# LDeakin/VkVolume

Hardware: AMD Instinct MI355X
Metric: Mray/s (higher is better)
Workload: dtype f32

## Files before the change

### vkvolume_amd/csrc/capi.hip

```cpp
#include <cmath>
#include <cstdarg>
#include <cstdio>
#include <cstdlib>
#include <cstring>
#include <dlfcn.h>
#include <mutex>
#include <new>

#include <algorithm>
#include <exception>
#include <string>
#include <vector>

#include "../host/load_volume.h"
#include "../host/vkv_math.hpp"
#include "vkv_device.hpp"
#include "../../include/vkvolume_amd_debug.h"

namespace vkv
{
int launch_gradient_map(vkv_ctx *, const uint8_t *, uint8_t *, VkvExtent3D, const VkvTransferFunctionUniform *, hipStream_t);
int launch_occupancy_map(vkv_ctx *, const uint8_t *, const uint8_t *, const uint8_t *, const VkvTransferFunctionUniform *, VkvExtent3D, uint8_t *,
                         VkvExtent3D, hipStream_t, uint32_t *d_bits, bool bits_ready = false);
int launch_distance_map(vkv_ctx *, uint8_t *, uint8_t *, VkvExtent3D, hipStream_t);
int launch_distance_map_anisotropic(vkv_ctx *, uint8_t *const[8], uint8_t *, VkvExtent3D, hipStream_t);
int launch_synth_volume(vkv_ctx *, uint8_t *, VkvExtent3D, uint32_t, uint32_t, hipStream_t);
int launch_scatter_tiles_frames(vkv_ctx *, uint32_t, void *const *, const void *const *, const VkvTileRect *, const uint32_t *, uint32_t, uint32_t, uint32_t, uint32_t, uint32_t,
                                uint32_t, hipStream_t);
void screen_tile_rect(const VkvRayCastUniform *, const VkvRayGen *, uint32_t, uint32_t, uint32_t, uint32_t, uint32_t, VkvTileRect *);
int prepare_render(vkv_ctx *, const VkvRenderParams *, uint32_t, hipStream_t);
// ... 93 lines not shown
			{
				void *q = nullptr;
				if (hipMalloc(&q, kScratchBytes) == hipSuccess)
				{
					ctx->overflow_scratch.push_back(q);
					p = static_cast<uint8_t *>(q);
				}
			}
			if (p)
			{
				b = new (std::nothrow) vkv_ctx::ScratchBlock;
				if (b)
				{
					b->p = p;
					ctx->scratch_blocks.emplace_back(b);
				}
			}
			if (!b)
			{
				set_error(ctx, VKV_E_UNSUPPORTED, "no scratch block left for a new stream: the arena reserves %zu (call vkv_prepare_render for the stream at set-up "
				                                  "time, give finished streams back with vkv_release_stream, or raise VKV_ARENA_BYTES)", ctx->table_base / kScratchBytes);
				return StreamScratch{};
			}
			ctx->scratch.emplace(key, b);
		}
	}
	StreamScratch r;
	r.lock = std::unique_lock<std::mutex>(b->lock);
	r.p    = b->p;
	return r;
}

static bool table_upload(vkv_ctx *ctx, vkv_ctx::Table &t, hipStream_t s, bool setup)
{
	const size_t bytes = t.host.size() * sizeof(uint32_t);
	bool         from_arena = false;
	t.d                = static_cast<uint32_t *>(arena_take_table(ctx, bytes, setup, &from_arena));
	if (!t.d)
		return false;
	if (hipEventCreateWithFlags(&t.uploaded, hipEventDisableTiming) != hipSuccess)
		return false;
	const void *src = t.host.data();
	if (from_arena && ctx->table_mirror)
	{
// ... 23 lines not shown
{
	if (t.ready)
		return t.d;
	if (setup ? hipEventSynchronize(t.uploaded) == hipSuccess : hipEventQuery(t.uploaded) == hipSuccess)
	{
		t.ready = true;
		return t.d;
	}
	if ((s != t.upload_stream || s == hipStreamPerThread) && hipStreamWaitEvent(s, t.uploaded, 0) != hipSuccess)
		return nullptr;
	return t.d;
}

constexpr size_t kMaxCachedTables = 1024;

const uint32_t *packed_addr_lut(vkv_ctx *ctx, int W, int H, int D, uint32_t *lut_y, uint32_t *lut_z, uint32_t *words, hipStream_t stream, bool setup)
{
	std::lock_guard<std::mutex> lock(ctx->mutex);
	for (auto *t : ctx->addr_luts)
		if (t->W == W && t->H == H && t->D == D)
		{
			*lut_y = t->lut_y, *lut_z = t->lut_z, *words = t->words;
			return table_on_stream(t->table, stream, setup);
		}
	if (ctx->addr_luts.size() >= kMaxCachedTables)
		return nullptr;
	const PackedDims pd  = packed_dims(W, H, D);
	const uint32_t   nmx = (uint32_t) (W + 1) / 32 + 1, nmy = (uint32_t) (H + 1) / 32 + 1, nmz = (uint32_t) (D + 1) / 32 + 1;
	const uint32_t   ny = 96 + nmx, nz = (ny + nmy + 1) & ~1u, total = nz + 2 * nmz;
	auto *           e  = new (std::nothrow) vkv_ctx::AddrLut{W, H, D, ny, nz, total, {}};
	if (!e)
		return nullptr;
	std::vector<uint32_t> &h = e->table.host;
	h.assign(total, 0u);
	for (uint32_t j = 0; j < 32; ++j)
	{
		h[j]      = (((j >> 2) & 7u) << 8) + (j & 3u) * 2u;
		h[32 + j] = (((j >> 2) & 7u) << 11) + (j & 3u) * 10u;
		h[64 + j] = (((j >> 2) & 7u) << 14) + (j & 3u) * 50u;
	}
	for (uint32_t m = 0; m < nmx; ++m)
		h[96 + m] = m << 17;
	for (uint32_t m = 0; m < nmy; ++m)
		h[ny + m] = (m * (uint32_t) pd.mx) << 17;
	for (uint32_t m = 0; m < nmz; ++m)
	{
		const uint64_t z = ((uint64_t) m * (uint64_t) pd.my * (uint64_t) pd.mx) << 17;
		h[nz + 2 * m] = (uint32_t) z, h[nz + 2 * m + 1] = (uint32_t) (z >> 32);
	}
	if (!table_upload(ctx, e->table, stream, setup))
	{
		delete e;
		return nullptr;
	}
	ctx->addr_luts.push_back(e);
	*lut_y = ny, *lut_z = nz, *words = total;
	return e->table.d;
}

const uint32_t *tile_start_order(vkv_ctx *ctx, uint32_t img_w, uint32_t img_h, uint32_t tile_w, uint32_t tile_h, uint32_t first, uint32_t stride, uint32_t count,
                                 hipStream_t stream, bool setup)
{
	if (count < 2)
		return nullptr;
	const uint32_t tiles_x = (img_w + tile_w - 1) / tile_w, tiles_y = (img_h + tile_h - 1) / tile_h;
	std::lock_guard<std::mutex> lock(ctx->mutex);
	const float mix_heavy_f = ctx->tuning.tile_mix_heavy, mix_spread_f = ctx->tuning.tile_mix_spread;
	for (auto *t : ctx->tile_orders)
		if (t->tiles_x == tiles_x && t->tiles_y == tiles_y && t->tile_w == tile_w && t->tile_h == tile_h && t->img_w == img_w && t->img_h == img_h && t->first == first &&
		    t->stride == stride && t->count == count && t->mix_heavy == mix_heavy_f && t->mix_spread == mix_spread_f)
			return table_on_stream(t->table, stream, setup);
// ... 282 lines not shown
			ctx->table_mirror = static_cast<uint8_t *>(m);
		void *cp = nullptr, *cd = nullptr;
		if (hipHostMalloc(&cp, (size_t) kCaptureSlots * kCaptureSlotBytes, hipHostMallocDefault) == hipSuccess &&
		    hipMalloc(&cd, (size_t) kCaptureSlots * kCaptureSlotBytes) == hipSuccess)
		{
			ctx->capture_pool = static_cast<uint8_t *>(cp), ctx->capture_pool_device = static_cast<uint8_t *>(cd);
			for (uint32_t i = 0; i < kCaptureSlots; ++i)
			{
				vkv_ctx::CaptureSlot c;
				c.pinned = ctx->capture_pool + (size_t) i * kCaptureSlotBytes, c.device = ctx->capture_pool_device + (size_t) i * kCaptureSlotBytes, c.pooled = true;
				ctx->capture_slots.push_back(c);
			}
		}
		else if (cp)
			(void) hipHostFree(cp);
	}
	*out_ctx      = ctx;
	return VKV_OK;
}

void vkv_destroy(vkv_ctx *ctx)
{
	if (!ctx)
		return;
	{
		DeviceGuard guard(ctx->device);
		(void) hipDeviceSynchronize();
		drop_tables(ctx);
		for (auto *f : ctx->feedback)
		{
			(void) hipFree(f->d_cost);
			(void) hipFree(f->d_order);
					delete f;
		}
		for (void *p : ctx->overflow_scratch)
			(void) hipFree(p);
		drop_capture_blocks(ctx);
		if (ctx->capture_pool)
			(void) hipHostFree(ctx->capture_pool);
		if (ctx->capture_pool_device)
			(void) hipFree(ctx->capture_pool_device);
		if (ctx->table_mirror)
			(void) hipHostFree(ctx->table_mirror);
		(void) hipFree(ctx->arena);
	}
	delete ctx;
}

int vkv_get_tuning(const vkv_ctx *ctx, VkvTuning *out)
{
	if (!ctx || !out)
		return VKV_E_INVALID_ARGUMENT;
// ... 680 lines not shown
	if (!P->d_out_color && !P->d_out_rgba8 && !P->d_out_counts && !P->d_out_depth)
		return set_error(ctx, VKV_E_INVALID_ARGUMENT, "render: no output buffer");
	return VKV_OK;
}

static void build_alpha_lut(const VkvTransferFunctionUniform &tf, float *lut)
{
	const float sf_inv = 1.0f / tf.sampling_factor;
	for (int a = 0; a < 256; ++a)
	{
		const float v = tf.voxel_alpha_factor * (1.0f - std::pow(1.0f - (float) a / 255.0f, sf_inv));
		lut[a]        = std::min(std::max(v, 0.0f), 1.0f);
	}
}

int vkv_render(vkv_ctx *ctx, const VkvRenderParams *P, void *stream)
{
	if (!ctx)
		return VKV_E_INVALID_ARGUMENT;
	DeviceGuard guard(ctx->device);
	const int   rc = check_render_params(ctx, P);
	if (rc != VKV_OK)
		return rc;
	float lut[256];
	build_alpha_lut(P->transfer_function, lut);
	return launch_render(ctx, P, lut, (hipStream_t) stream);
}

int vkv_render_batch(vkv_ctx *ctx, const VkvRenderParams *P, uint32_t count, void *stream)
{
	if (!ctx)
		return VKV_E_INVALID_ARGUMENT;
	DeviceGuard guard(ctx->device);
	if (!P || count == 0 || count > VKV_MAX_BATCH)
		return set_error(ctx, VKV_E_INVALID_ARGUMENT, "render_batch: count must be 1 .. %d", VKV_MAX_BATCH);
	std::vector<float> luts((size_t) count * 256);
	for (uint32_t i = 0; i < count; ++i)
	{
		const int rc = check_render_params(ctx, &P[i]);
		if (rc != VKV_OK)
			return rc;
		const VkvRenderParams &a = P[i], &b = P[0];
		if (a.options.skipping_type != b.options.skipping_type || (a.options.early_ray_termination != 0) != (b.options.early_ray_termination != 0) ||
		    (a.transfer_function.use_gradient != 0) != (b.transfer_function.use_gradient != 0) ||
		    (a.use_precomputed_gradient != 0) != (b.use_precomputed_gradient != 0))
			return set_error(ctx, VKV_E_INVALID_ARGUMENT, "render_batch: frame %u needs a different kernel variant than frame 0", i);
		build_alpha_lut(a.transfer_function, luts.data() + (size_t) i * 256);
	}
	return launch_render_batch(ctx, P, count, luts.data(), (hipStream_t) stream);
}

static bool resolve_rect(const VkvTileRect *rect, uint32_t image_width, uint32_t image_height, uint32_t tile_width, uint32_t tile_height, VkvTileRect &out)
{
	const uint32_t tiles_x = (image_width + tile_width - 1) / tile_width, tiles_y = (image_height + tile_height - 1) / tile_height;
	if (!rect || rect->w == 0 || rect->h == 0)
	{
		out = VkvTileRect{0u, 0u, tiles_x, tiles_y};
		return true;
	}
	out = *rect;
	return (uint64_t) rect->x0 + rect->w <= tiles_x && (uint64_t) rect->y0 + rect->h <= tiles_y;
}
// ... 224 lines not shown
```

### vkvolume_amd/csrc/raymarch.hip

```cpp
#include <algorithm>
#include <cmath>
#include <cstdio>
#include <cstdlib>
#include <cstring>
#include <mutex>
#include <new>
#include <vector>

#include "raymarch_inst.hpp"

constexpr int kCostBins = 1024;

__device__ __forceinline__ void tile_order_from_cost(uint32_t *__restrict__ cost, uint32_t *__restrict__ order_out, uint32_t count)
{
	__shared__ uint32_t s_bin[kCostBins];
	constexpr int       kPerThread = 40;
	for (int b = threadIdx.x; b < kCostBins; b += blockDim.x)
		s_bin[b] = 0;
	__syncthreads();
	for (uint32_t base = 0; base < count; base += 256u * kPerThread)
	{
		uint32_t c[kPerThread];
#pragma unroll
		for (int j = 0; j < kPerThread; ++j)
// ... 83 lines not shown
	if (A.order_out)
		tile_order_from_cost(A.tile_cost, A.order_out, A.tile_count);
}

namespace vkv
{

LeanChoice choose_lean(const RayMarchArgs &a, const VkvTuning &T)
{
	const size_t lut_bytes = (size_t) a.lut_words * sizeof(uint32_t);
	if (!a.packed || !a.addr_lut || lut_bytes > kMaxLutBytes || !map_fits_u24((uint32_t) a.mw, (uint32_t) a.mh, (uint32_t) a.md))
		return {0, lean_lds_bytes(0, 0, a.W, a.H, a.D)};
	const bool        no_full  = T.address_tables < 2;
	const size_t      full_end = kFullLutWord * 4 + full_lut_bytes(a.W, a.H, a.D);
	const bool        fits_u32 = packed_bytes(packed_dims(a.W, a.H, a.D)) <= (1ull << 33);
	if (!no_full && fits_u32 && full_end <= (size_t) T.full_table_lds_limit)
		return {2, lean_lds_bytes(2, a.lut_words, a.W, a.H, a.D)};
	return {1, lean_lds_bytes(1, a.lut_words, a.W, a.H, a.D)};
}

static int launch_single(vkv_ctx *ctx, int skip, bool ert, int sched, const VkvTuning &T, int grad, RayMarchArgs &a, hipStream_t s)
{
	switch (skip)
	{
		case VKV_SKIP_NONE: return ert ? RayMarchLaunchers<VKV_SKIP_NONE, true>::single(ctx, sched, T, grad, a, s) : RayMarchLaunchers<VKV_SKIP_NONE, false>::single(ctx, sched, T, grad, a, s);
		case VKV_SKIP_BLOCK: return ert ? RayMarchLaunchers<VKV_SKIP_BLOCK, true>::single(ctx, sched, T, grad, a, s) : RayMarchLaunchers<VKV_SKIP_BLOCK, false>::single(ctx, sched, T, grad, a, s);
		case VKV_SKIP_DISTANCE: return ert ? RayMarchLaunchers<VKV_SKIP_DISTANCE, true>::single(ctx, sched, T, grad, a, s) : RayMarchLaunchers<VKV_SKIP_DISTANCE, false>::single(ctx, sched, T, grad, a, s);
		case VKV_SKIP_ANISOTROPIC_DISTANCE:
			return ert ? RayMarchLaunchers<VKV_SKIP_ANISOTROPIC_DISTANCE, true>::single(ctx, sched, T, grad, a, s) : RayMarchLaunchers<VKV_SKIP_ANISOTROPIC_DISTANCE, false>::single(ctx, sched, T, grad, a, s);
		default: return set_error(ctx, VKV_E_INVALID_ARGUMENT, "render: bad skipping_type %d", skip);
	}
// ... 218 lines not shown
	a.back        = (int) std::ceil(P->transfer_function.sampling_factor);
	a.clamp_always = T.clamp_always != 0 ? 1u : 0u;
	{
		double vx = 0.0, vy = 0.0;
		const double dim[3] = {(double) a.W, (double) a.H, (double) a.D};
		for (int k = 0; k < 3; ++k)
			vx += (double) a.ddx[k] * dim[k] * (double) a.ddx[k] * dim[k], vy += (double) a.ddy[k] * dim[k] * (double) a.ddy[k] * dim[k];
		const double r = (vx > 0.0 && vy > 0.0) ? std::sqrt(vx / vy) : 1.0;
		a.wave_pw_log2 = T.wave_shape == 4 ? 2u : (T.wave_shape == 8 ? 3u : (T.wave_shape == 16 ? 4u : (r >= 1.6 ? 2u : (r <= 1.0 / 1.6 ? 4u : 3u))));
	}
	{
		const float m[3] = {(float) a.mw, (float) a.mh, (float) a.md};
		for (int k = 0; k < 3; ++k)
			a.mapf[k] = m[k], a.mapb[k] = std::nextafterf(m[k], 0.0f);
	}
	a.addr_lut = nullptr, a.lut_y = a.lut_z = a.lut_words = 0;
	if (a.packed && T.address_tables != 0)
		a.addr_lut = packed_addr_lut(ctx, a.W, a.H, a.D, &a.lut_y, &a.lut_z, &a.lut_words, s, setup);
	screen_bound_of_box(a, T);
	a.tile_order = (T.tile_order_linear || !whole_schedule) ? nullptr
	                                                         : tile_start_order(ctx, a.img_w, a.img_h, a.tile_w, a.tile_h, a.tile_first, a.tile_stride, a.tile_count, s, setup);
	a.order_h = 0;
	if (!whole_schedule && !T.tile_order_linear && a.tile_first == 0 && a.tile_stride == 1 && (uint64_t) a.tile_count == (uint64_t) a.tiles_x * P->tiles.rect.h)
		a.order_h = P->tiles.rect.h;
	for (int i = 0; i < 256; ++i)
		a.alpha_lut[i] = alpha_lut[i];
	return VKV_OK;
}

static bool apply_feedback(vkv_ctx *ctx, RayMarchArgs &a, hipStream_t s)
{
	(void) s;
	const void *      target = a.out_rgba8 ? (const void *) a.out_rgba8 : (const void *) a.out_color;
// ... 96 lines not shown
			rc = fill_render_args(ctx, &P[i], lut, a, s, T, true, true);
		if (rc != VKV_OK)
			return rc;
		load_render_code(P[i].options.skipping_type, P[i].options.early_ray_termination != 0);
	}
	load_feedback_code();
	if (!stream_scratch(ctx, s, true).p)
		return VKV_E_UNSUPPORTED;
	return VKV_OK;
}

int launch_render_batch(vkv_ctx *ctx, const VkvRenderParams *P, uint32_t n, const float *alpha_luts, hipStream_t s)
{
	static_assert(kMaxBatch * sizeof(RayMarchArgs) <= kScratchBytes - kBatchArgsOffset, "batch argument blocks must fit the stream scratch");
	static_assert(kPullHeadsBytes + kMaxBatch * sizeof(RayMarchArgs) <= kCaptureSlotBytes, "a captured launch's upload must fit its pinned slot");
	const VkvTuning           T = tuning_of(ctx);
	std::vector<RayMarchArgs> host(n);
	for (uint32_t i = 0; i < n; ++i)
	{
		const int rc = fill_render_args(ctx, &P[i], alpha_luts + (size_t) i * 256, host[i], s, T, false, true);
		if (rc != VKV_OK)
			return rc;
		if (!host[i].packed)
			return set_error(ctx, VKV_E_INVALID_ARGUMENT, "render_batch: frame %u has no packed sampling image (d_packed_volume)", i);
		if (host[i].blocks_per_tile != host[0].blocks_per_tile)
			return set_error(ctx, VKV_E_INVALID_ARGUMENT, "render_batch: frame %u has a different tile size than frame 0", i);
		if (ctx->d_debug_orders && i < ctx->debug_order_frames && ctx->debug_order_count == host[i].tile_count)
			host[i].tile_order = ctx->d_debug_orders + (size_t) i * ctx->debug_order_count;
	}
	uint32_t max_tiles = 0, ref = 0;
	bool     same_count = true;
	for (uint32_t i = n; i-- > 0;)
	{
		max_tiles = std::max(max_tiles, host[i].nblocks ? host[i].tile_count : 0u);
		if (host[i].nblocks)
			ref = i;
	}
	if (max_tiles == 0)
		return VKV_OK;
	for (uint32_t i = 0; i < n; ++i)
		same_count = same_count && host[i].nblocks != 0 && host[i].tile_count == max_tiles;
	bool any_sort = false;
	for (uint32_t i = 0; i < n && P[0].options.early_ray_termination != 0; ++i)
		any_sort = apply_feedback(ctx, host[i], s) || any_sort;
	const StreamScratch scratch = stream_scratch(ctx, s);
	if (!scratch.p)
		return VKV_E_UNSUPPORTED;
	RayMarchArgs *   d_frames = reinterpret_cast<RayMarchArgs *>(scratch.p + kBatchArgsOffset);
	uint32_t *       d_heads  = reinterpret_cast<uint32_t *>(scratch.p + kBatchArgsOffset - kPullHeadsBytes);
	std::vector<uint8_t> upload(kPullHeadsBytes + n * sizeof(RayMarchArgs), 0);
	std::memcpy(upload.data() + kPullHeadsBytes, host.data(), n * sizeof(RayMarchArgs));
	const void *upload_src = upload.data();
	struct SlotGuard
	{
		vkv_ctx *ctx;
		size_t   index;
		bool     armed;
		~SlotGuard()
		{
			if (!armed)
				return;
			std::lock_guard<std::mutex> lock(ctx->mutex);
			if (index < ctx->capture_slots.size())
				ctx->capture_slots[index].in_use = false, ctx->capture_slots[index].owner = VkvStreamKey{};
		}
	} slot_guard{ctx, 0, false};
	{
		hipStreamCaptureStatus capture = hipStreamCaptureStatusNone;
		if (hipStreamIsCapturing(s, &capture) == hipSuccess && capture == hipStreamCaptureStatusActive)
		{
			std::lock_guard<std::mutex> lock(ctx->mutex);
			vkv_ctx::CaptureSlot *      slot = nullptr;
			for (auto &c : ctx->capture_slots)
				if (!c.in_use)
				{
					slot = &c;
					break;
				}
			if (!slot)
			{
				vkv_ctx::CaptureSlot c;
				void *               hp = nullptr, *dp = nullptr;
				hipStreamCaptureMode mode = hipStreamCaptureModeRelaxed;
				(void) hipThreadExchangeStreamCaptureMode(&mode);
				const hipError_t ea = hipHostMalloc(&hp, kCaptureSlotBytes, hipHostMallocDefault);
				const hipError_t eb = ea == hipSuccess ? hipMalloc(&dp, kCaptureSlotBytes) : ea;
				const bool failed = ea != hipSuccess || eb != hipSuccess || !hp || !dp;
				if (failed && hp)
					(void) hipHostFree(hp);
				(void) hipThreadExchangeStreamCaptureMode(&mode);
				if (failed)
					return set_error(ctx, VKV_E_UNSUPPORTED, "render_batch: no argument block for a captured launch: %s", hipGetErrorString(ea != hipSuccess ? ea : eb));
				c.pinned = static_cast<uint8_t *>(hp), c.device = static_cast<uint8_t *>(dp);
				ctx->capture_slots.push_back(c);
				slot = &ctx->capture_slots.back();
			}
			slot->in_use = true, slot->owner = stream_key(s);
			slot_guard.index = (size_t) (slot - ctx->capture_slots.data()), slot_guard.armed = true;
			std::memcpy(slot->pinned, upload.data(), upload.size());
			upload_src = slot->pinned;
			d_heads    = reinterpret_cast<uint32_t *>(slot->device);
			d_frames   = reinterpret_cast<RayMarchArgs *>(slot->device + kPullHeadsBytes);
		}
	}
	const hipError_t e = hipMemcpyAsync(d_heads, upload_src, upload.size(), hipMemcpyHostToDevice, s);
	if (e != hipSuccess)
		return set_error(ctx, (int) e, "render_batch: argument upload: %s", hipGetErrorString(e));
	const uint64_t grid = (uint64_t) ((max_tiles + 7u) / 8u) * 8u * host[0].blocks_per_tile * n;
	if (grid > 0x7fffffffull)
		return set_error(ctx, VKV_E_UNSUPPORTED, "render_batch: too many workgroups for one launch");
	const bool ert  = P[0].options.early_ray_termination != 0;
	const int  grad = !P[0].transfer_function.use_gradient ? 0 : (P[0].use_precomputed_gradient ? 1 : 2);
	const bool        sequential = T.batch_sequential != 0;
	const uint32_t    gpf        = sequential ? (uint32_t) (grid / n / 8) : 0u;
	LeanChoice        choice     = choose_lean(host[ref], T);
	bool              no_counts  = true;
	for (uint32_t i = 0; i < n; ++i)
		no_counts = no_counts && (host[i].nblocks == 0 || !wants_counts(host[i]));
	for (uint32_t i = 0; i < n; ++i)
	{
		if (i == ref || host[i].nblocks == 0)
			continue;
// ... 33 lines not shown
```

### vkvolume_amd/csrc/raymarch_core.hpp

```cpp
#pragma once

#include <type_traits>

#include "vkv_device.hpp"

using namespace vkv;

constexpr int kTraceWords = 10;
constexpr uint32_t kFillPerTile = 3;

struct RayMarchArgs
{
	float dir00[3], ddx[3], ddy[3];
	float cam[3];
	float plane_tex[4];
	float block_size[3];
	float model[16], view[16], proj[16];
	float view_proj_inv[16], model_inv[16];
	float sampling_factor, grad_modifier;
	int W, H, D, mw, mh, md;
	const uint8_t * vol, *grad, *tf;
	const uint8_t * packed;
	int             pmx, pmy;
	const uint32_t *tf_bits;
// ... 5 lines not shown
	const float *   in_depth;
	uint32_t        depth_attachment, blend;
	uint32_t        img_w, img_h, tile_w, tile_h, tiles_x, tile_first, tile_stride, tile_count, compact;
	uint32_t        org_x, org_y;
	uint32_t        fill_tiles, img_tiles_x, rect_tx0, rect_ty0, rect_th;
	uint32_t        fill_rgba8_rows;
	uint32_t        blocks_per_tile_x, blocks_per_tile, nblocks;
	int             test;
	unsigned long long *trace;
	int             back;
	uint32_t        clamp_always;
	float           mapf[3], mapb[3];
	uint32_t        wave_pw_log2;
	const uint32_t *addr_lut;
	uint32_t        lut_y, lut_z, lut_words;
	uint32_t        cull_x0, cull_x1, cull_y0, cull_y1;
	const uint32_t *tile_order;
	uint32_t        order_h;
	uint32_t *      queue_heads;
	uint32_t *      tile_cost;
	uint32_t *      order_out;
	float           alpha_lut[256];
};

struct Ray
{
	float          ex, ey, ez;
	float          sx, sy, sz;
	float          six, siy, siz;
	const uint8_t *dmap;
// ... 697 lines not shown
			float    unorm[256];
		} g;
		struct
		{
			float  ai[258], ag[258];
			float2 pair[256];
		} s;
	};
};

__device__ __forceinline__ bool tf_is_separable(const RayMarchArgs &A)
{
	return A.tf_bits != nullptr && (A.tf_bits[kTfFlagWord] & kTfFlagSeparable) != 0u;
}

__device__ __forceinline__ bool stage_tables_er(const RayMarchArgs &A, RmLds &L)
{
	const bool sep = tf_is_separable(A);
	for (int i = threadIdx.x; i < 256; i += blockDim.x)
	{
		const float a = A.alpha_lut[i];
		if (!sep)
			L.g.alpha[i] = a;
		if (sep)
		{
			L.s.ai[i]   = __uint_as_float(A.tf_bits[kTfAiWord + i]);
			L.s.ag[i]   = __uint_as_float(A.tf_bits[kTfAgWord + i]);
			if (i == 255)
				L.s.ai[256] = L.s.ai[255], L.s.ag[256] = L.s.ag[255];
			L.s.pair[i] = i == 0 ? make_float2(0.0f, 0.0f) : make_float2(a, unorm8(i) * a);
		}
		else
			L.g.unorm[i] = unorm8(i);
	}
	if (!sep && A.tf_bits)
		for (int i = threadIdx.x; i < 2048; i += blockDim.x)
			L.g.bits[i] = A.tf_bits[i];
	__syncthreads();
	return sep;
}
template <int W>
__device__ __forceinline__ bool block_pixel(const RayMarchArgs &A, uint32_t b, uint32_t rb, uint32_t &px, uint32_t &py, uint32_t &o)
{
	constexpr uint32_t G = 64 / W;
	uint32_t           bx, by;
	const uint32_t     wb = rb / G, g = rb % G;
	if (W == 1)
	{
		const uint32_t pwl = A.wave_pw_log2, pprl = 4u - pwl;
		bx = ((wb & ((1u << pprl) - 1u)) << pwl) + (g & ((1u << pwl) - 1u));
		by = ((wb >> pprl) << (6u - pwl)) + (g >> pwl);
	}
	else
// ... 163 lines not shown
}

constexpr uint32_t kFullLutWord  = 1028;
__host__ __device__ __forceinline__ bool map_fits_u24(uint32_t mw, uint32_t mh, uint32_t md) { return (uint64_t) mh * md < (1ull << 24) && mw < (1u << 24); }
constexpr size_t   kFullLdsLimit = 17920;

__host__ __device__ __forceinline__ size_t full_lut_bytes(int W, int H, int D) { return (size_t) (W + 2 + H + 2 + D + 2) * 4; }

__host__ __forceinline__ size_t lean_lds_bytes(int kind, uint32_t lut_words, int W, int H, int D)
{
	const size_t two_level = kLdsBase + sizeof(RmLds) + (size_t) lut_words * 4;
	if (kind == 0)
		return kLdsBase + sizeof(RmLds);
	if (kind == 1)
		return two_level;
	const size_t full_end = kLdsBase + (size_t) kFullLutWord * 4 + full_lut_bytes(W, H, D);
	return two_level > full_end ? two_level : full_end;
}

__device__ __forceinline__ uint32_t *full_lut_base(const RmLds &L) { return const_cast<uint32_t *>(reinterpret_cast<const uint32_t *>(&L)) + kFullLutWord; }

__device__ __forceinline__ void stage_full_lut(const RayMarchArgs &A, RmLds &L)
{
	static_assert(sizeof(((RmLds *) nullptr)->s) == kFullLutWord * 4, "full tables start behind the separable TF tables");
	const uint32_t  nx = (uint32_t) A.W + 2u, ny = (uint32_t) A.H + 2u, nz = (uint32_t) A.D + 2u;
	uint32_t *      fx = full_lut_base(L), *fy = fx + nx, *fz = fy + ny;
	const uint32_t *g  = A.addr_lut;
	for (uint32_t b = threadIdx.x; b < nx; b += blockDim.x)
		fx[b] = (g[b & 31u] + g[kLutXm + (b >> 5)]) >> 1;
	for (uint32_t b = threadIdx.x; b < ny; b += blockDim.x)
		fy[b] = (g[32u + (b & 31u)] + g[A.lut_y + (b >> 5)]) >> 1;
	for (uint32_t b = threadIdx.x; b < nz; b += blockDim.x)
		fz[b] = (uint32_t) ((((((uint64_t) g[A.lut_z + 2u * (b >> 5) + 1u]) << 32) | g[A.lut_z + 2u * (b >> 5)]) + g[64u + (b & 31u)]) >> 1);
}

struct FullLutConsts
{
	float          w, h, d, oy, oz;
	const uint8_t *base;
};

template <bool SCALAR = false>
__device__ __forceinline__ FullLutConsts full_lut_consts(const RayMarchArgs &A)
{
	FullLutConsts c;
	c.w = (float) A.W, c.h = (float) A.H, c.d = (float) A.D;
	c.base = A.packed;
	c.oy = (float) (4 * (A.W + 2) + 4);
// ... 482 lines not shown
	R.o = o;
	const unsigned long long t_start = A.trace ? __builtin_amdgcn_s_memrealtime() : 0ull;
	const unsigned long long c_start = A.trace ? __builtin_amdgcn_s_memtime() : 0ull;
	bool marched = false;
	if (inside)
	{
		if (px >= A.cull_x0 && px <= A.cull_x1 && py >= A.cull_y0 && py <= A.cull_y1)
			marched = ray_setup<SKIP>(A, px, py, R);
		else
			ray_clear(R);
	}
	uint32_t  iter  = 0;
	LeanStamp stamp = {};
	if (wg_any(marched))
	{
		if ((LF & kLeanLut) != 0 && PACKED && GRAD != 2)
		{
			if ((LF & kLeanFull) != 0 && tf_is_separable(A))
				stage_full_lut(A, L);
			else
				stage_addr_lut(A);
		}
		const bool sep = stage_tables_er(A, L);
		if (marched)
		{
			if (sep)
			{
				constexpr bool kSafe = (LF & kLeanSafe) != 0 && (LF & kLeanFull) != 0 && PACKED && GRAD != 2 && SKIP != VKV_SKIP_NONE && (LF & kLeanStamp) == 0;
				if constexpr (kSafe)
				{
					if (lean_free_wave(A, R))
						lean_march<SKIP, ERT, GRAD, PACKED, true, LF, true>(A, R, L, iter, stamp);
					else
						lean_march<SKIP, ERT, GRAD, PACKED, true, LF>(A, R, L, iter, stamp);
				}
				else
					lean_march<SKIP, ERT, GRAD, PACKED, true, LF>(A, R, L, iter, stamp);
			}
// ... 138 lines not shown
				rec[0] = t_start, rec[1] = t_end, rec[2] = it, rec[3] = ((unsigned long long) __builtin_amdgcn_s_getreg((3 << 11) | 20) << 32) | (rank * upt + w);
				rec[4] = t_setup, rec[5] = t_march;
				for (int x = 6; x < kTraceWords; ++x)
					rec[x] = 0;
			}
		}
	}
}

template <int SKIP, bool ERT, int GRAD, uint32_t LF>
__global__ void __launch_bounds__(256) __attribute__((amdgpu_waves_per_eu(8, 8))) k_raymarch_lean_pull(const RayMarchArgs *__restrict__ frames, uint32_t n, uint32_t *__restrict__ heads)
{
	lean_lds_check();
	RmLds &             L  = lean_lds();
	const RayMarchArgs &A0 = frames[0];
	if ((LF & kLeanLut) != 0 && GRAD != 2)
	{
		if ((LF & kLeanFull) != 0 && tf_is_separable(A0))
			stage_full_lut(A0, L);
		else
			stage_addr_lut(A0);
	}
	if (stage_tables_er(A0, L))
		pull_units<SKIP, ERT, GRAD, LF, true>(frames, n, heads, L);
	else
		pull_units<SKIP, ERT, GRAD, LF, false>(frames, n, heads, L);
}

namespace vkv
{
int fill_render_args(vkv_ctx *ctx, const VkvRenderParams *P, const float *alpha_lut, RayMarchArgs &a, hipStream_t s, const VkvTuning &T, bool setup, bool batch);
}
```

### vkvolume_amd/csrc/vkv_device.hpp

```cpp
#pragma once

#include <hip/hip_runtime.h>
#include <stdint.h>

#include <map>
#include <memory>
#include <mutex>
#include <thread>
#include <unordered_map>
#include <vector>

#include "../../include/vkvolume_amd.h"

namespace vkv
{

__device__ __forceinline__ float g_min(float x, float y) { return (y < x) ? y : x; }
__device__ __forceinline__ float g_max(float x, float y) { return (x < y) ? y : x; }
__device__ __forceinline__ float g_clamp(float x, float lo, float hi) { return g_min(g_max(x, lo), hi); }
__device__ __forceinline__ float g_step(float edge, float x) { return (x < edge) ? 0.0f : 1.0f; }
__device__ __forceinline__ float g_sign(float x) { return (x > 0.0f) ? 1.0f : ((x < 0.0f) ? -1.0f : 0.0f); }
__device__ __forceinline__ int   i_clamp(int x, int lo, int hi) { return min(max(x, lo), hi); }

constexpr float kInv255 = 1.0f / 255.0f;
// ... 138 lines not shown
	uint8_t *           arena = nullptr;
	size_t              arena_bytes = 0;
	size_t              table_base = 0;
	size_t              scratch_used = 0, table_used = 0;
	uint8_t *           table_mirror = nullptr;
	std::vector<void *> overflow;
	std::vector<void *> overflow_scratch;
	struct CaptureSlot
	{
		uint8_t *   pinned = nullptr, *device = nullptr;
		VkvStreamKey owner;
		bool         in_use = false, pooled = false;
	};
	uint8_t *                capture_pool = nullptr, *capture_pool_device = nullptr;
	std::vector<CaptureSlot> capture_slots;
	struct ScratchBlock
	{
		uint8_t *  p = nullptr;
		std::mutex lock;
	};
	std::vector<std::unique_ptr<ScratchBlock>> scratch_blocks;
	std::map<VkvStreamKey, ScratchBlock *>     scratch;
	std::vector<ScratchBlock *>                free_scratch;
	struct Table
	{
		std::vector<uint32_t> host;
		uint32_t *            d = nullptr;
		hipEvent_t            uploaded = nullptr;
		hipStream_t           upload_stream = nullptr;
		bool                  ready = false;
	};
	struct TileOrder
	{
		uint32_t tiles_x, tiles_y, tile_w, tile_h, img_w, img_h, first, stride, count;
		float    mix_heavy, mix_spread;
		Table    table;
	};
	std::vector<TileOrder *> tile_orders;
	struct AddrLut
	{
		int      W, H, D;
		uint32_t lut_y, lut_z, words;
		Table    table;
	};
	std::vector<AddrLut *> addr_luts;
	struct TileFeedback
	{
		const void *target;
		uint32_t    img_w, img_h, tile_w, tile_h, first, stride, count;
		uint32_t    org_x, org_y, tiles_x;
		uint32_t *  d_cost, *d_order;
		bool        has_cost;
		uint32_t    frames;
		uint32_t    measured_at = 0;
		uint32_t    period = 8;
		uint32_t    used = 0;
		float       view_dir[3] = {0, 0, 0}, view_pos[3] = {0, 0, 0};
// ... 1 lines not shown
		bool        has_prev = false;
	};
	std::vector<TileFeedback *> feedback;
};

namespace vkv
{
int  set_error(vkv_ctx *ctx, int code, const char *fmt, ...);
int  check_launch(vkv_ctx *ctx, const char *what);
int  check_box(vkv_ctx *ctx, const char *what, VkvExtent3D extent, const VkvBox *box);
VkvStreamKey stream_key(hipStream_t stream);
struct StreamScratch
{
	uint8_t *                    p = nullptr;
	std::unique_lock<std::mutex> lock;
};
StreamScratch stream_scratch(vkv_ctx *ctx, hipStream_t stream, bool setup = false);
const uint32_t *packed_addr_lut(vkv_ctx *ctx, int W, int H, int D, uint32_t *lut_y, uint32_t *lut_z, uint32_t *words, hipStream_t stream, bool setup = false);
const uint32_t *tile_start_order(vkv_ctx *ctx, uint32_t img_w, uint32_t img_h, uint32_t tile_w, uint32_t tile_h, uint32_t first, uint32_t stride, uint32_t count,
                                 hipStream_t stream, bool setup = false);
VkvTuning tuning_of(vkv_ctx *ctx);
constexpr size_t kScratchBytes     = 128 * 1024;
constexpr size_t kScratchReserve   = 16;
constexpr uint32_t kCaptureSlots   = 32;
constexpr size_t   kCaptureSlotBytes = 96 * 1024;
constexpr uint32_t kMaxDynamicLds  = 64 * 1024 - 1024;
constexpr size_t kTfBitsOffset     = 0;
constexpr size_t kQueueHeadsOffset = 8192 + 64;
constexpr size_t kTfRangesOffset   = 16 * 1024;
constexpr size_t kPullHeadsBytes   = 2048;
constexpr uint32_t kPullHeadStride = 64;
constexpr size_t kBatchArgsOffset  = 32 * 1024 + kPullHeadsBytes;
constexpr uint32_t kMaxBatch       = VKV_MAX_BATCH;
static_assert(kTfRangesOffset >= kQueueHeadsOffset + 32 && kTfRangesOffset + 4 * 2048 * 8 <= kScratchBytes, "the range table must fit the scratch block");

struct DeviceGuard
{
	int  prev = -1;
	bool switched = false;
// ... 15 lines not shown
```

Baseline: 21150.

## Precompute full address tables on host, cache alpha LUTs, pin batch argument uploads

The full per-axis address tables are now built once on the host and stored after the packed LUT. Kernels copy them into LDS with vectorized 16-byte loads, issued before the TF-table staging so the two overlap, instead of recomputing each entry from the two-level tables. Alpha LUTs are cached per context and deduplicated within a batch. Batch argument uploads now go through a per-stream pinned ring with events rather than a pageable vector. The cost is more host memory, more state and a larger device table. Per-workgroup prologue work also drops.

```diff
diff --git a/vkvolume_amd/csrc/addr_tables.hpp b/vkvolume_amd/csrc/addr_tables.hpp
--- /dev/null
+++ b/vkvolume_amd/csrc/addr_tables.hpp
@@ -0,0 +1,52 @@
+#pragma once
+
+#include <stdint.h>
+
+#include <vector>
+
+namespace vkv
+{
+struct AddrTables
+{
+	uint32_t lut_y = 0, lut_z = 0, words = 0;
+	uint32_t full = 0, full_words = 0;
+};
+
+inline AddrTables build_addr_tables(int W, int H, int D, int mx, int my, bool with_full, std::vector<uint32_t> &h)
+{
+	AddrTables     t;
+	const uint32_t nmx = (uint32_t) (W + 1) / 32 + 1, nmy = (uint32_t) (H + 1) / 32 + 1, nmz = (uint32_t) (D + 1) / 32 + 1;
+	const uint32_t ny = 96 + nmx, nz = (ny + nmy + 1) & ~1u, total = nz + 2 * nmz;
+	t.lut_y = ny, t.lut_z = nz, t.words = total;
+	const uint32_t nx_full = (uint32_t) W + 2u, ny_full = (uint32_t) H + 2u, nz_full = (uint32_t) D + 2u;
+	if (with_full)
+		t.full = (total + 3u) & ~3u, t.full_words = (nx_full + ny_full + nz_full + 3u) & ~3u;
+	h.assign((size_t) (with_full ? t.full + t.full_words : total), 0u);
+	for (uint32_t j = 0; j < 32; ++j)
+	{
+		h[j]      = (((j >> 2) & 7u) << 8) + (j & 3u) * 2u;
+		h[32 + j] = (((j >> 2) & 7u) << 11) + (j & 3u) * 10u;
+		h[64 + j] = (((j >> 2) & 7u) << 14) + (j & 3u) * 50u;
+	}
+	for (uint32_t m = 0; m < nmx; ++m)
+		h[96 + m] = m << 17;
+	for (uint32_t m = 0; m < nmy; ++m)
+		h[ny + m] = (m * (uint32_t) mx) << 17;
+	for (uint32_t m = 0; m < nmz; ++m)
+	{
+		const uint64_t z = ((uint64_t) m * (uint64_t) my * (uint64_t) mx) << 17;
+		h[nz + 2 * m] = (uint32_t) z, h[nz + 2 * m + 1] = (uint32_t) (z >> 32);
+	}
+	if (with_full)
+	{
+		uint32_t *fx = h.data() + t.full, *fy = fx + nx_full, *fz = fy + ny_full;
+		for (uint32_t b = 0; b < nx_full; ++b)
+			fx[b] = (h[b & 31u] + h[96u + (b >> 5)]) >> 1;
+		for (uint32_t b = 0; b < ny_full; ++b)
+			fy[b] = (h[32u + (b & 31u)] + h[ny + (b >> 5)]) >> 1;
+		for (uint32_t b = 0; b < nz_full; ++b)
+			fz[b] = (uint32_t) ((((((uint64_t) h[nz + 2u * (b >> 5) + 1u]) << 32) | h[nz + 2u * (b >> 5)]) + h[64u + (b & 31u)]) >> 1);
+	}
+	return t;
+}
+}
diff --git a/vkvolume_amd/csrc/capi.hip b/vkvolume_amd/csrc/capi.hip
--- a/vkvolume_amd/csrc/capi.hip
+++ b/vkvolume_amd/csrc/capi.hip
@@ -14,6 +14,7 @@
 
 #include "../host/load_volume.h"
 #include "../host/vkv_math.hpp"
+#include "addr_tables.hpp"
 #include "vkv_device.hpp"
 #include "../../include/vkvolume_amd_debug.h"
 
@@ -137,6 +138,16 @@
 				{
 					b->p = p;
 					ctx->scratch_blocks.emplace_back(b);
+					const size_t index = (size_t) (p - ctx->arena) / kScratchBytes;
+					if (ctx->upload_pool && p >= ctx->arena && index < kScratchReserve)
+						for (uint32_t k = 0; k < vkv_ctx::kUploadRing; ++k)
+						{
+							vkv_ctx::UploadSlot &u = b->upload[k];
+							if (hipEventCreateWithFlags(&u.done, hipEventDisableTiming) == hipSuccess)
+								u.pinned = ctx->upload_pool + (index * vkv_ctx::kUploadRing + k) * kUploadSlotBytes;
+							else
+								u.done = nullptr;
+						}
 				}
 			}
 			if (!b)
@@ -149,8 +160,9 @@
 		}
 	}
 	StreamScratch r;
-	r.lock = std::unique_lock<std::mutex>(b->lock);
-	r.p    = b->p;
+	r.lock  = std::unique_lock<std::mutex>(b->lock);
+	r.p     = b->p;
+	r.block = b;
 	return r;
 }
 
@@ -204,47 +216,31 @@
 
 constexpr size_t kMaxCachedTables = 1024;
 
-const uint32_t *packed_addr_lut(vkv_ctx *ctx, int W, int H, int D, uint32_t *lut_y, uint32_t *lut_z, uint32_t *words, hipStream_t stream, bool setup)
+const uint32_t *packed_addr_lut(vkv_ctx *ctx, int W, int H, int D, uint32_t *lut_y, uint32_t *lut_z, uint32_t *words, uint32_t *full, hipStream_t stream, bool setup)
 {
 	std::lock_guard<std::mutex> lock(ctx->mutex);
 	for (auto *t : ctx->addr_luts)
 		if (t->W == W && t->H == H && t->D == D)
 		{
-			*lut_y = t->lut_y, *lut_z = t->lut_z, *words = t->words;
+			*lut_y = t->lut_y, *lut_z = t->lut_z, *words = t->words, *full = t->full;
 			return table_on_stream(t->table, stream, setup);
 		}
 	if (ctx->addr_luts.size() >= kMaxCachedTables)
 		return nullptr;
-	const PackedDims pd  = packed_dims(W, H, D);
-	const uint32_t   nmx = (uint32_t) (W + 1) / 32 + 1, nmy = (uint32_t) (H + 1) / 32 + 1, nmz = (uint32_t) (D + 1) / 32 + 1;
-	const uint32_t   ny = 96 + nmx, nz = (ny + nmy + 1) & ~1u, total = nz + 2 * nmz;
-	auto *           e  = new (std::nothrow) vkv_ctx::AddrLut{W, H, D, ny, nz, total, {}};
+	const PackedDims pd = packed_dims(W, H, D);
+	const bool       with_full = packed_bytes(pd) <= (1ull << 33) && ((size_t) W + 2 + (size_t) H + 2 + (size_t) D + 2) * 4 <= kMaxDynamicLds;
+	auto *           e = new (std::nothrow) vkv_ctx::AddrLut{W, H, D, 0, 0, 0, 0, {}};
 	if (!e)
 		return nullptr;
-	std::vector<uint32_t> &h = e->table.host;
-	h.assign(total, 0u);
-	for (uint32_t j = 0; j < 32; ++j)
-	{
-		h[j]      = (((j >> 2) & 7u) << 8) + (j & 3u) * 2u;
-		h[32 + j] = (((j >> 2) & 7u) << 11) + (j & 3u) * 10u;
-		h[64 + j] = (((j >> 2) & 7u) << 14) + (j & 3u) * 50u;
-	}
-	for (uint32_t m = 0; m < nmx; ++m)
-		h[96 + m] = m << 17;
-	for (uint32_t m = 0; m < nmy; ++m)
-		h[ny + m] = (m * (uint32_t) pd.mx) << 17;
-	for (uint32_t m = 0; m < nmz; ++m)
-	{
-		const uint64_t z = ((uint64_t) m * (uint64_t) pd.my * (uint64_t) pd.mx) << 17;
-		h[nz + 2 * m] = (uint32_t) z, h[nz + 2 * m + 1] = (uint32_t) (z >> 32);
-	}
+	const AddrTables t = build_addr_tables(W, H, D, pd.mx, pd.my, with_full, e->table.host);
+	e->lut_y = t.lut_y, e->lut_z = t.lut_z, e->words = t.words, e->full = t.full;
 	if (!table_upload(ctx, e->table, stream, setup))
 	{
 		delete e;
 		return nullptr;
 	}
 	ctx->addr_luts.push_back(e);
-	*lut_y = ny, *lut_z = nz, *words = total;
+	*lut_y = e->lut_y, *lut_z = e->lut_z, *words = e->words, *full = e->full;
 	return e->table.d;
 }
 
@@ -557,6 +553,9 @@
 		}
 		else if (cp)
 			(void) hipHostFree(cp);
+		void *up = nullptr;
+		if (hipHostMalloc(&up, kScratchReserve * vkv_ctx::kUploadRing * kUploadSlotBytes, hipHostMallocDefault) == hipSuccess)
+			ctx->upload_pool = static_cast<uint8_t *>(up);
 	}
 	*out_ctx      = ctx;
 	return VKV_OK;
@@ -579,6 +578,12 @@
 		for (void *p : ctx->overflow_scratch)
 			(void) hipFree(p);
 		drop_capture_blocks(ctx);
+		for (auto &b : ctx->scratch_blocks)
+			for (auto &u : b->upload)
+				if (u.done)
+					(void) hipEventDestroy(u.done);
+		if (ctx->upload_pool)
+			(void) hipHostFree(ctx->upload_pool);
 		if (ctx->capture_pool)
 			(void) hipHostFree(ctx->capture_pool);
 		if (ctx->capture_pool_device)
@@ -1289,6 +1294,30 @@
 	}
 }
 
+static void cached_alpha_lut(vkv_ctx *ctx, const VkvTransferFunctionUniform &tf, float *lut)
+{
+	uint32_t factor_bits, sampling_bits;
+	std::memcpy(&factor_bits, &tf.voxel_alpha_factor, 4), std::memcpy(&sampling_bits, &tf.sampling_factor, 4);
+	{
+		std::lock_guard<std::mutex> lock(ctx->mutex);
+		for (const auto &e : ctx->alpha_luts)
+			if (e.factor_bits == factor_bits && e.sampling_bits == sampling_bits)
+			{
+				std::memcpy(lut, e.lut, sizeof(e.lut));
+				return;
+			}
+	}
+	build_alpha_lut(tf, lut);
+	vkv_ctx::AlphaLut e;
+	e.factor_bits = factor_bits, e.sampling_bits = sampling_bits;
+	std::memcpy(e.lut, lut, sizeof(e.lut));
+	std::lock_guard<std::mutex> lock(ctx->mutex);
+	if (ctx->alpha_luts.size() < kAlphaLuts)
+		ctx->alpha_luts.push_back(e);
+	else
+		ctx->alpha_luts[ctx->alpha_next++ % kAlphaLuts] = e;
+}
+
 int vkv_render(vkv_ctx *ctx, const VkvRenderParams *P, void *stream)
 {
 	if (!ctx)
@@ -1298,7 +1327,7 @@
 	if (rc != VKV_OK)
 		return rc;
 	float lut[256];
-	build_alpha_lut(P->transfer_function, lut);
+	cached_alpha_lut(ctx, P->transfer_function, lut);
 	return launch_render(ctx, P, lut, (hipStream_t) stream);
 }
 
@@ -1320,7 +1349,15 @@
 		    (a.transfer_function.use_gradient != 0) != (b.transfer_function.use_gradient != 0) ||
 		    (a.use_precomputed_gradient != 0) != (b.use_precomputed_gradient != 0))
 			return set_error(ctx, VKV_E_INVALID_ARGUMENT, "render_batch: frame %u needs a different kernel variant than frame 0", i);
-		build_alpha_lut(a.transfer_function, luts.data() + (size_t) i * 256);
+		uint32_t same = i;
+		for (uint32_t j = 0; j < i && same == i; ++j)
+			if (std::memcmp(&P[j].transfer_function.voxel_alpha_factor, &a.transfer_function.voxel_alpha_factor, 4) == 0 &&
+			    std::memcmp(&P[j].transfer_function.sampling_factor, &a.transfer_function.sampling_factor, 4) == 0)
+				same = j;
+		if (same != i)
+			std::memcpy(luts.data() + (size_t) i * 256, luts.data() + (size_t) same * 256, 256 * sizeof(float));
+		else
+			cached_alpha_lut(ctx, a.transfer_function, luts.data() + (size_t) i * 256);
 	}
 	return launch_render_batch(ctx, P, count, luts.data(), (hipStream_t) stream);
 }
diff --git a/vkvolume_amd/csrc/raymarch.hip b/vkvolume_amd/csrc/raymarch.hip
--- a/vkvolume_amd/csrc/raymarch.hip
+++ b/vkvolume_amd/csrc/raymarch.hip
@@ -121,7 +121,7 @@
 	const bool        no_full  = T.address_tables < 2;
 	const size_t      full_end = kFullLutWord * 4 + full_lut_bytes(a.W, a.H, a.D);
 	const bool        fits_u32 = packed_bytes(packed_dims(a.W, a.H, a.D)) <= (1ull << 33);
-	if (!no_full && fits_u32 && full_end <= (size_t) T.full_table_lds_limit)
+	if (!no_full && fits_u32 && a.lut_full != 0 && full_end <= (size_t) T.full_table_lds_limit)
 		return {2, lean_lds_bytes(2, a.lut_words, a.W, a.H, a.D)};
 	return {1, lean_lds_bytes(1, a.lut_words, a.W, a.H, a.D)};
 }
@@ -370,9 +370,9 @@
 		for (int k = 0; k < 3; ++k)
 			a.mapf[k] = m[k], a.mapb[k] = std::nextafterf(m[k], 0.0f);
 	}
-	a.addr_lut = nullptr, a.lut_y = a.lut_z = a.lut_words = 0;
+	a.addr_lut = nullptr, a.lut_y = a.lut_z = a.lut_words = a.lut_full = 0;
 	if (a.packed && T.address_tables != 0)
-		a.addr_lut = packed_addr_lut(ctx, a.W, a.H, a.D, &a.lut_y, &a.lut_z, &a.lut_words, s, setup);
+		a.addr_lut = packed_addr_lut(ctx, a.W, a.H, a.D, &a.lut_y, &a.lut_z, &a.lut_words, &a.lut_full, s, setup);
 	screen_bound_of_box(a, T);
 	a.tile_order = (T.tile_order_linear || !whole_schedule) ? nullptr
 	                                                         : tile_start_order(ctx, a.img_w, a.img_h, a.tile_w, a.tile_h, a.tile_first, a.tile_stride, a.tile_count, s, setup);
@@ -499,8 +499,35 @@
 {
 	static_assert(kMaxBatch * sizeof(RayMarchArgs) <= kScratchBytes - kBatchArgsOffset, "batch argument blocks must fit the stream scratch");
 	static_assert(kPullHeadsBytes + kMaxBatch * sizeof(RayMarchArgs) <= kCaptureSlotBytes, "a captured launch's upload must fit its pinned slot");
-	const VkvTuning           T = tuning_of(ctx);
-	std::vector<RayMarchArgs> host(n);
+	static_assert(kPullHeadsBytes + kMaxBatch * sizeof(RayMarchArgs) <= kUploadSlotBytes, "a launch's upload must fit a slot of the block's pinned ring");
+	const VkvTuning     T = tuning_of(ctx);
+	const StreamScratch scratch = stream_scratch(ctx, s);
+	if (!scratch.p)
+		return VKV_E_UNSUPPORTED;
+	hipStreamCaptureStatus capture = hipStreamCaptureStatusNone;
+	const bool             capturing = hipStreamIsCapturing(s, &capture) == hipSuccess && capture == hipStreamCaptureStatusActive;
+	const size_t          upload_bytes = kPullHeadsBytes + n * sizeof(RayMarchArgs);
+	vkv_ctx::UploadSlot * ring_slot = nullptr;
+	for (uint32_t k = 0; k < vkv_ctx::kUploadRing && !capturing && !ring_slot; ++k)
+	{
+		vkv_ctx::UploadSlot &u = scratch.block->upload[(scratch.block->upload_next + k) % vkv_ctx::kUploadRing];
+		if (!u.pinned)
+			continue;
+		if (u.pending && hipEventQuery(u.done) == hipSuccess)
+			u.pending = false;
+		if (!u.pending)
+		{
+			ring_slot                  = &u;
+			scratch.block->upload_next = (scratch.block->upload_next + k + 1) % vkv_ctx::kUploadRing;
+		}
+	}
+	(void) hipGetLastError();
+	std::vector<uint8_t> pageable;
+	if (!ring_slot)
+		pageable.resize(upload_bytes);
+	uint8_t *const upload = ring_slot ? ring_slot->pinned : pageable.data();
+	std::memset(upload, 0, upload_bytes);
+	RayMarchArgs *const host = reinterpret_cast<RayMarchArgs *>(upload + kPullHeadsBytes);
 	for (uint32_t i = 0; i < n; ++i)
 	{
 		const int rc = fill_render_args(ctx, &P[i], alpha_luts + (size_t) i * 256, host[i], s, T, false, true);
@@ -528,14 +555,9 @@
 	bool any_sort = false;
 	for (uint32_t i = 0; i < n && P[0].options.early_ray_termination != 0; ++i)
 		any_sort = apply_feedback(ctx, host[i], s) || any_sort;
-	const StreamScratch scratch = stream_scratch(ctx, s);
-	if (!scratch.p)
-		return VKV_E_UNSUPPORTED;
 	RayMarchArgs *   d_frames = reinterpret_cast<RayMarchArgs *>(scratch.p + kBatchArgsOffset);
 	uint32_t *       d_heads  = reinterpret_cast<uint32_t *>(scratch.p + kBatchArgsOffset - kPullHeadsBytes);
-	std::vector<uint8_t> upload(kPullHeadsBytes + n * sizeof(RayMarchArgs), 0);
-	std::memcpy(upload.data() + kPullHeadsBytes, host.data(), n * sizeof(RayMarchArgs));
-	const void *upload_src = upload.data();
+	const void *upload_src = upload;
 	struct SlotGuard
 	{
 		vkv_ctx *ctx;
@@ -551,8 +573,7 @@
 		}
 	} slot_guard{ctx, 0, false};
 	{
-		hipStreamCaptureStatus capture = hipStreamCaptureStatusNone;
-		if (hipStreamIsCapturing(s, &capture) == hipSuccess && capture == hipStreamCaptureStatusActive)
+		if (capturing)
 		{
 			std::lock_guard<std::mutex> lock(ctx->mutex);
 			vkv_ctx::CaptureSlot *      slot = nullptr;
@@ -582,15 +603,22 @@
 			}
 			slot->in_use = true, slot->owner = stream_key(s);
 			slot_guard.index = (size_t) (slot - ctx->capture_slots.data()), slot_guard.armed = true;
-			std::memcpy(slot->pinned, upload.data(), upload.size());
+			std::memcpy(slot->pinned, upload, upload_bytes);
 			upload_src = slot->pinned;
 			d_heads    = reinterpret_cast<uint32_t *>(slot->device);
 			d_frames   = reinterpret_cast<RayMarchArgs *>(slot->device + kPullHeadsBytes);
 		}
 	}
-	const hipError_t e = hipMemcpyAsync(d_heads, upload_src, upload.size(), hipMemcpyHostToDevice, s);
+	const hipError_t e = hipMemcpyAsync(d_heads, upload_src, upload_bytes, hipMemcpyHostToDevice, s);
 	if (e != hipSuccess)
 		return set_error(ctx, (int) e, "render_batch: argument upload: %s", hipGetErrorString(e));
+	if (ring_slot)
+	{
+		if (hipEventRecord(ring_slot->done, s) == hipSuccess)
+			ring_slot->pending = true;
+		else
+			(void) hipStreamSynchronize(s);
+	}
 	const uint64_t grid = (uint64_t) ((max_tiles + 7u) / 8u) * 8u * host[0].blocks_per_tile * n;
 	if (grid > 0x7fffffffull)
 		return set_error(ctx, VKV_E_UNSUPPORTED, "render_batch: too many workgroups for one launch");
diff --git a/vkvolume_amd/csrc/raymarch_core.hpp b/vkvolume_amd/csrc/raymarch_core.hpp
--- a/vkvolume_amd/csrc/raymarch_core.hpp
+++ b/vkvolume_amd/csrc/raymarch_core.hpp
@@ -43,6 +43,7 @@
 	uint32_t        wave_pw_log2;
 	const uint32_t *addr_lut;
 	uint32_t        lut_y, lut_z, lut_words;
+	uint32_t        lut_full;
 	uint32_t        cull_x0, cull_x1, cull_y0, cull_y1;
 	const uint32_t *tile_order;
 	uint32_t        order_h;
@@ -770,9 +771,11 @@
 	return A.tf_bits != nullptr && (A.tf_bits[kTfFlagWord] & kTfFlagSeparable) != 0u;
 }
 
-__device__ __forceinline__ bool stage_tables_er(const RayMarchArgs &A, RmLds &L)
+__device__ __forceinline__ bool stage_tables_er(const RayMarchArgs &A, RmLds &L, bool sync = true)
 {
 	const bool sep = tf_is_separable(A);
+	typedef const __attribute__((address_space(1))) uint32_t *global_u32_ptr;
+	const global_u32_ptr tf_words = (global_u32_ptr) (uintptr_t) A.tf_bits;
 	for (int i = threadIdx.x; i < 256; i += blockDim.x)
 	{
 		const float a = A.alpha_lut[i];
@@ -780,10 +783,10 @@
 			L.g.alpha[i] = a;
 		if (sep)
 		{
-			L.s.ai[i]   = __uint_as_float(A.tf_bits[kTfAiWord + i]);
-			L.s.ag[i]   = __uint_as_float(A.tf_bits[kTfAgWord + i]);
+			const float ai = __uint_as_float(tf_words[kTfAiWord + i]), ag = __uint_as_float(tf_words[kTfAgWord + i]);
+			L.s.ai[i] = ai, L.s.ag[i] = ag;
 			if (i == 255)
-				L.s.ai[256] = L.s.ai[255], L.s.ag[256] = L.s.ag[255];
+				L.s.ai[256] = ai, L.s.ag[256] = ag;
 			L.s.pair[i] = i == 0 ? make_float2(0.0f, 0.0f) : make_float2(a, unorm8(i) * a);
 		}
 		else
@@ -792,7 +795,8 @@
 	if (!sep && A.tf_bits)
 		for (int i = threadIdx.x; i < 2048; i += blockDim.x)
 			L.g.bits[i] = A.tf_bits[i];
-	__syncthreads();
+	if (sync)
+		__syncthreads();
 	return sep;
 }
 template <int W>
@@ -986,24 +990,53 @@
 		return kLdsBase + sizeof(RmLds);
 	if (kind == 1)
 		return two_level;
-	const size_t full_end = kLdsBase + (size_t) kFullLutWord * 4 + full_lut_bytes(W, H, D);
+	const size_t full_end = kLdsBase + (size_t) kFullLutWord * 4 + ((full_lut_bytes(W, H, D) + 15u) & ~(size_t) 15u);
 	return two_level > full_end ? two_level : full_end;
 }
 
 __device__ __forceinline__ uint32_t *full_lut_base(const RmLds &L) { return const_cast<uint32_t *>(reinterpret_cast<const uint32_t *>(&L)) + kFullLutWord; }
 
+typedef uint32_t lut_v4u __attribute__((ext_vector_type(4)));
+constexpr uint32_t kFullCopyRounds = 4;
+static_assert((kLdsBase + kFullLutWord * 4) % 16 == 0, "the full tables are written with 16-byte LDS stores");
+static_assert(kFullLdsLimit - kFullLutWord * 4 <= kFullCopyRounds * 256 * 16, "the unrolled rounds cover the tables of the default LDS limit");
+
+struct FullLutCopy
+{
+	lut_v4u  r[kFullCopyRounds];
+	uint32_t nvec;
+};
+
+__device__ __forceinline__ FullLutCopy full_lut_issue(const RayMarchArgs &A)
+{
+	typedef const __attribute__((address_space(1))) lut_v4u *global_v4u_ptr;
+	FullLutCopy          c;
+	const global_v4u_ptr g = (global_v4u_ptr) (uintptr_t) (A.addr_lut + A.lut_full);
+	c.nvec                 = ((uint32_t) (A.W + 2 + A.H + 2 + A.D + 2) + 3u) >> 2;
+#pragma unroll
+	for (uint32_t k = 0; k < kFullCopyRounds; ++k)
+		c.r[k] = g[min(threadIdx.x + k * blockDim.x, c.nvec - 1u)];
+	return c;
+}
+
+__device__ __forceinline__ void full_lut_commit(const RayMarchArgs &A, const FullLutCopy &c, RmLds &L)
+{
+	static_assert(sizeof(((RmLds *) nullptr)->s) == kFullLutWord * 4, "full tables start behind the separable TF tables");
+	typedef const __attribute__((address_space(1))) lut_v4u *global_v4u_ptr;
+	lut_v4u *dst = reinterpret_cast<lut_v4u *>(full_lut_base(L));
+#pragma unroll
+	for (uint32_t k = 0; k < kFullCopyRounds; ++k)
+		if (threadIdx.x + k * blockDim.x < c.nvec)
+			dst[threadIdx.x + k * blockDim.x] = c.r[k];
+	const global_v4u_ptr g = (global_v4u_ptr) (uintptr_t) (A.addr_lut + A.lut_full);
+	for (uint32_t i = threadIdx.x + kFullCopyRounds * blockDim.x; i < c.nvec; i += blockDim.x)
+		dst[i] = g[i];
+}
+
 __device__ __forceinline__ void stage_full_lut(const RayMarchArgs &A, RmLds &L)
 {
-	static_assert(sizeof(((RmLds *) nullptr)->s) == kFullLutWord * 4, "full tables start behind the separable TF tables");
-	const uint32_t  nx = (uint32_t) A.W + 2u, ny = (uint32_t) A.H + 2u, nz = (uint32_t) A.D + 2u;
-	uint32_t *      fx = full_lut_base(L), *fy = fx + nx, *fz = fy + ny;
-	const uint32_t *g  = A.addr_lut;
-	for (uint32_t b = threadIdx.x; b < nx; b += blockDim.x)
-		fx[b] = (g[b & 31u] + g[kLutXm + (b >> 5)]) >> 1;
-	for (uint32_t b = threadIdx.x; b < ny; b += blockDim.x)
-		fy[b] = (g[32u + (b & 31u)] + g[A.lut_y + (b >> 5)]) >> 1;
-	for (uint32_t b = threadIdx.x; b < nz; b += blockDim.x)
-		fz[b] = (uint32_t) ((((((uint64_t) g[A.lut_z + 2u * (b >> 5) + 1u]) << 32) | g[A.lut_z + 2u * (b >> 5)]) + g[64u + (b & 31u)]) >> 1);
+	const FullLutCopy c = full_lut_issue(A);
+	full_lut_commit(A, c, L);
 }
 
 struct FullLutConsts
@@ -1516,14 +1549,20 @@
 	LeanStamp stamp = {};
 	if (wg_any(marched))
 	{
-		if ((LF & kLeanLut) != 0 && PACKED && GRAD != 2)
-		{
-			if ((LF & kLeanFull) != 0 && tf_is_separable(A))
-				stage_full_lut(A, L);
-			else
+		bool sep;
+		if ((LF & kLeanLut) != 0 && (LF & kLeanFull) != 0 && PACKED && GRAD != 2 && tf_is_separable(A))
+		{
+			const FullLutCopy c = full_lut_issue(A);
+			sep                 = stage_tables_er(A, L, false);
+			full_lut_commit(A, c, L);
+			__syncthreads();
+		}
+		else
+		{
+			if ((LF & kLeanLut) != 0 && PACKED && GRAD != 2)
 				stage_addr_lut(A);
-		}
-		const bool sep = stage_tables_er(A, L);
+			sep = stage_tables_er(A, L);
+		}
 		if (marched)
 		{
 			if (sep)
@@ -1692,14 +1731,21 @@
 	lean_lds_check();
 	RmLds &             L  = lean_lds();
 	const RayMarchArgs &A0 = frames[0];
-	if ((LF & kLeanLut) != 0 && GRAD != 2)
-	{
-		if ((LF & kLeanFull) != 0 && tf_is_separable(A0))
-			stage_full_lut(A0, L);
-		else
+	bool sep;
+	if ((LF & kLeanLut) != 0 && (LF & kLeanFull) != 0 && GRAD != 2 && tf_is_separable(A0))
+	{
+		const FullLutCopy c = full_lut_issue(A0);
+		sep                 = stage_tables_er(A0, L, false);
+		full_lut_commit(A0, c, L);
+		__syncthreads();
+	}
+	else
+	{
+		if ((LF & kLeanLut) != 0 && GRAD != 2)
 			stage_addr_lut(A0);
-	}
-	if (stage_tables_er(A0, L))
+		sep = stage_tables_er(A0, L);
+	}
+	if (sep)
 		pull_units<SKIP, ERT, GRAD, LF, true>(frames, n, heads, L);
 	else
 		pull_units<SKIP, ERT, GRAD, LF, false>(frames, n, heads, L);
diff --git a/vkvolume_amd/csrc/vkv_device.hpp b/vkvolume_amd/csrc/vkv_device.hpp
--- a/vkvolume_amd/csrc/vkv_device.hpp
+++ b/vkvolume_amd/csrc/vkv_device.hpp
@@ -176,11 +176,28 @@
 	};
 	uint8_t *                capture_pool = nullptr, *capture_pool_device = nullptr;
 	std::vector<CaptureSlot> capture_slots;
+	struct UploadSlot
+	{
+		uint8_t *  pinned = nullptr;
+		hipEvent_t done = nullptr;
+		bool       pending = false;
+	};
+	static constexpr uint32_t kUploadRing = 4;
 	struct ScratchBlock
 	{
 		uint8_t *  p = nullptr;
 		std::mutex lock;
-	};
+		UploadSlot upload[kUploadRing];
+		uint32_t   upload_next = 0;
+	};
+	uint8_t *upload_pool = nullptr;
+	struct AlphaLut
+	{
+		uint32_t factor_bits, sampling_bits;
+		float    lut[256];
+	};
+	std::vector<AlphaLut> alpha_luts;
+	uint32_t              alpha_next = 0;
 	std::vector<std::unique_ptr<ScratchBlock>> scratch_blocks;
 	std::map<VkvStreamKey, ScratchBlock *>     scratch;
 	std::vector<ScratchBlock *>                free_scratch;
@@ -203,6 +220,7 @@
 	{
 		int      W, H, D;
 		uint32_t lut_y, lut_z, words;
+		uint32_t full;
 		Table    table;
 	};
 	std::vector<AddrLut *> addr_luts;
@@ -234,15 +252,18 @@
 {
 	uint8_t *                    p = nullptr;
 	std::unique_lock<std::mutex> lock;
+	vkv_ctx::ScratchBlock *      block = nullptr;
 };
 StreamScratch stream_scratch(vkv_ctx *ctx, hipStream_t stream, bool setup = false);
-const uint32_t *packed_addr_lut(vkv_ctx *ctx, int W, int H, int D, uint32_t *lut_y, uint32_t *lut_z, uint32_t *words, hipStream_t stream, bool setup = false);
+const uint32_t *packed_addr_lut(vkv_ctx *ctx, int W, int H, int D, uint32_t *lut_y, uint32_t *lut_z, uint32_t *words, uint32_t *full, hipStream_t stream, bool setup = false);
 const uint32_t *tile_start_order(vkv_ctx *ctx, uint32_t img_w, uint32_t img_h, uint32_t tile_w, uint32_t tile_h, uint32_t first, uint32_t stride, uint32_t count,
                                  hipStream_t stream, bool setup = false);
 VkvTuning tuning_of(vkv_ctx *ctx);
 constexpr size_t kScratchBytes     = 128 * 1024;
 constexpr size_t kScratchReserve   = 16;
 constexpr uint32_t kCaptureSlots   = 32;
+constexpr size_t   kUploadSlotBytes = 64 * 1024;
+constexpr size_t   kAlphaLuts = 8;
 constexpr size_t   kCaptureSlotBytes = 96 * 1024;
 constexpr uint32_t kMaxDynamicLds  = 64 * 1024 - 1024;
 constexpr size_t kTfBitsOffset     = 0;
```

Measured after the change: 22290 (median of 6 runs). +5.4%, better.
